# Roy-Shubhajit/FIT-GNN

Measured on AMD Instinct MI355X. Metric: edges aggregated/sec (GCN fwd+bwd) on coarsened subgraphs, higher is better.
Workload: dtype f32

## Files before the change

fit-gnn_amd/csrc/gcn_ops.hip:

```cpp
#include <hip/hip_runtime.h>
#include <stdint.h>

#include <algorithm>

#include "common.h"
#include "fitgnn_hip.h"

namespace {

__global__ void gcn_deg_kernel(const int32_t *__restrict__ rowptr, const float *__restrict__ w, float *__restrict__ dinv,
                               int32_t n_rows) {
    const int i = blockIdx.x * blockDim.x + threadIdx.x;
    if (i >= n_rows) return;
    const int e0 = rowptr[i], e1 = rowptr[i + 1];
    float d = 0.f;
    if (w) {
        for (int e = e0; e < e1; ++e) d += w[e];
    } else {
        d = (float)(e1 - e0);
    }
    dinv[i] = d > 0.f ? 1.0f / sqrtf(d) : 0.f;
}

__global__ void gcn_val_kernel(const int32_t *__restrict__ rowptr, const int32_t *__restrict__ col,
// ... 228 lines not shown
        for (int c = ph; c < n_chunks; c += kColsumPhases) s += partial[(int64_t)c * H + h];
    }
    red[ph][cl] = s;
    __syncthreads();
    for (int w = kColsumPhases / 2; w >= 1; w >>= 1) {
        if (ph < w) red[ph][cl] = red[ph][cl] + red[ph + w][cl];
        __syncthreads();
    }
    if (ph == 0 && h < H) {
        if (db2 && h >= split) db2[h - split] = red[0][cl];
        else if (tr_rows > 0 && h < tr_rows * tr_cols) db[(h % tr_cols) * tr_rows + h / tr_cols] = red[0][cl];
        else db[h] = red[0][cl];
    }
}

__global__ __launch_bounds__(256) void sum_leading_kernel(const float4 *__restrict__ part, int32_t B, int64_t W4,
                                                          float4 *__restrict__ out) {
    const int64_t i = (int64_t)blockIdx.x * 256 + threadIdx.x;
    if (i >= W4) return;
    float4 s[4];
#pragma unroll
    for (int k = 0; k < 4; ++k) s[k] = make_float4(0.f, 0.f, 0.f, 0.f);
    int b = 0;
    for (; b + 4 <= B; b += 4) {
#pragma unroll
        for (int k = 0; k < 4; ++k) {
            const float4 v = part[(int64_t)(b + k) * W4 + i];
            s[k].x += v.x; s[k].y += v.y; s[k].z += v.z; s[k].w += v.w;
        }
    }
// ... 634 lines not shown
    const int blocks = std::min(256, (n_rows + 255) / 256);
    const int rows_per_block = (n_rows + blocks - 1) / blocks;
    const int lds = (kRowTile * row_tile_pitch(C) + 256) * (int)sizeof(float);
    static std::atomic<uint64_t> lds_done{0};
    if (const int rc = fitgnn_lds_limit_once((const void *)narrow_colsum_kernel, (kRowTile * row_tile_pitch(kNarrowMaxC) + 256) * (int)sizeof(float), lds_done)) return rc;
    hipLaunchKernelGGL(narrow_colsum_kernel, dim3(blocks), dim3(256), lds, s, x, ldx, n_rows, C, rows_per_block, (float *)work);
    hipLaunchKernelGGL(colsum_partials_kernel, dim3((C + kColsumCols - 1) / kColsumCols), dim3(kColsumPhases * kColsumCols), 0, s,
                       (const float *)work, blocks, C, out);
    return (int)hipGetLastError();
}

extern "C" int fitgnn_colsum_partials_f32(const float *partial, int32_t n_chunks, int32_t H, float *out, void *stream) {
    if (n_chunks < 1 || H < 1 || !partial || !out) return FITGNN_E_BADARG;
    hipLaunchKernelGGL(colsum_partials_kernel, dim3((H + kColsumCols - 1) / kColsumCols), dim3(kColsumPhases * kColsumCols), 0,
                       (hipStream_t)stream, partial, n_chunks, H, out);
    return (int)hipGetLastError();
}

extern "C" int fitgnn_sum_leading_f32(const float *part, int32_t B, int64_t W, float *out, void *stream) {
    if (B < 1 || W < 0 || (W % 4) != 0) return FITGNN_E_BADARG;
    if (W == 0) return 0;
    if (!part || !out) return FITGNN_E_BADARG;
    if ((((uintptr_t)part | (uintptr_t)out) % 16) != 0) return FITGNN_E_ALIGN;
    const int64_t W4 = W / 4;
    hipLaunchKernelGGL(sum_leading_kernel, dim3((unsigned)((W4 + 255) / 256)), dim3(256), 0, (hipStream_t)stream,
                       (const float4 *)part, B, W4, (float4 *)out);
    return (int)hipGetLastError();
}

extern "C" int fitgnn_gcn_norm_csr_f32(const int32_t *rowptr, const int32_t *col, const float *w, float *val,
// ... 180 lines not shown
```

fit-gnn_amd/csrc/tile_plan.hip:

```cpp
#include <stdint.h>

#include <algorithm>
#include <vector>

#include "fitgnn_hip.h"

namespace {

struct Planner {
    const int32_t *rowptr, *col;
    int32_t max_rows, max_window;
    fitgnn_tile_t *tiles;
    int32_t *win_cols, *lcol;
    int32_t nt = 0, nw = 0;
    std::vector<int32_t> stamp, slot, cur;

    void emit_contiguous(int32_t r0, int32_t r1, int32_t c0, int32_t wn) {
        fitgnn_tile_t t;
        t.row_begin = r0; t.row_end = r1; t.win_begin = c0; t.win_rows = wn;
        t.nnz_begin = rowptr[r0]; t.nnz_end = rowptr[r1];
        t.reserved[0] = 0; t.reserved[1] = 0;
        for (int32_t e = rowptr[r0]; e < rowptr[r1]; ++e) {
            const int32_t s = col[e] - c0;
            lcol[e] = (s >= 0 && s < wn) ? s : -(col[e] + 1);
// ... 146 lines not shown
        rec[0] = (int32_t)r0; rec[1] = (int32_t)r1; rec[2] = rowptr[r0]; rec[3] = rowptr[r1];
        rec[4] = (int32_t)nlong; rec[6] = rec[7] = 0;
        int32_t cnt = 0;
        for (int64_t r = r0; r < r1; ++r)
            if (rowptr[r + 1] - rowptr[r] > long_row) {
                if (nlong >= long_capacity) return FITGNN_E_WORKSPACE;
                long_rows[nlong++] = (int32_t)r;
                ++cnt;
            }
        rec[5] = cnt;
        ++b;
    }
    *n_tiles = nt; *n_large = nl; *n_long = nlong;
    return 0;
}
```

fit-gnn_amd/fitgnn_amd/_lib.py:

```python
import ctypes
import os

_HERE = os.path.dirname(os.path.abspath(__file__))
LIB_PATH = os.path.join(os.path.dirname(_HERE), "lib", "libfitgnn_hip.so")

c_i32, c_i64, c_u32, c_u64, c_f32, c_size = (ctypes.c_int32, ctypes.c_int64, ctypes.c_uint32, ctypes.c_uint64,
                                              ctypes.c_float, ctypes.c_size_t)
ptr = ctypes.c_void_p

EPI_BIAS, EPI_ELU, EPI_DROPOUT, EPI_SEED_DEVICE = 1, 2, 4, 8
SPMM_GATHER = 0x100
MAX_K = 16
MATCH_HEAVY_EDGE, MATCH_ALGEBRAIC_JC = 0, 1
MATCH_SMALL_MAX_NODES, MATCH_SMALL_MAX_NNZ, MATCH_SMALL_MAX_K, MATCH_SMALL_LDS_BUDGET = 128, 1024, 12, 65536
MATCH_DONE, MATCH_TOO_BIG, MATCH_BAD_INPUT = 1, 2, 3
QUALITY_MAX_K = 64

SIGNATURES = {
    "fitgnn_abi_version": (ctypes.c_int, []),
    "fitgnn_error_string": (ctypes.c_char_p, [ctypes.c_int]),
    "fitgnn_stream_copy_f32": (ctypes.c_int, [ptr, ptr, c_i64, ptr]),
    "fitgnn_spmm_default_window_rows": (ctypes.c_int, []),
    "fitgnn_spmm_max_window_rows": (ctypes.c_int, [c_i32]),
    "fitgnn_gcn_norm_csr_f32": (ctypes.c_int, [ptr, ptr, ptr, ptr, ptr, c_i32, ptr]),
# ... 16 lines not shown
    "fitgnn_spmm_csr_stream_dz_f32": (ctypes.c_int, [ptr, ptr, ptr, c_i64, ptr, c_i64, ptr, c_i64, c_i32, c_i32, ptr, c_i32, ptr, c_i32, ptr, ptr,
                                                     ptr, c_u32, c_f32, c_u64, ptr, ptr, ptr]),
    "fitgnn_spmm_rows_compact_parts": (c_i32, [c_i32]),
    "fitgnn_spmm_rows_compact_f32": (ctypes.c_int, [ptr, ptr, ptr, c_i64, ptr, c_i64, c_i32, ptr, c_i64, c_i32, c_i32, ptr]),
    "fitgnn_spmm_rows_compact_dz_f32": (ctypes.c_int, [ptr, ptr, ptr, c_i64, ptr, c_i64, c_i32, ptr, c_i64, c_i32, c_i32, ptr, c_u32, c_f32,
                                                       c_u64, ptr, ptr, ptr]),
    "fitgnn_two_hop_rows_f32": (ctypes.c_int, [ptr, ptr, ptr, ptr, c_i64, c_i32, ptr, c_i32, ptr, c_i32, c_u32, c_f32, c_u64, ptr, ptr, c_i64, ptr]),
    "fitgnn_spmm_two_hop_blocks_f32": (ctypes.c_int, [ptr, ptr, ptr, ptr, c_i64, ptr, c_i64, c_i32, c_i32, ptr, c_i32, ptr, ptr, ptr, ptr, ptr, c_i64,
                                                      c_i32, ptr, ptr, c_u32, c_f32, c_u64, ptr, ptr, ptr]),
    "fitgnn_segment_sum_f32": (ctypes.c_int, [ptr, ptr, c_i32, ptr, c_i64, c_i32, ptr, c_i64, ptr]),
    "fitgnn_segment_max_f32": (ctypes.c_int, [ptr, ptr, c_i32, ptr, c_i64, c_i32, ptr, ptr, ptr]),
    "fitgnn_segment_max_bwd_f32": (ctypes.c_int, [ptr, ptr, c_i32, c_i32, ptr, c_i64, ptr]),
    "fitgnn_segment_expand_f32": (ctypes.c_int, [ptr, ptr, ptr, c_i64, c_i32, ptr, ptr]),
    "fitgnn_make_tiles_host": (ctypes.c_int, [ptr, c_i64, c_i32, ptr, c_i64, ptr]),
    "fitgnn_split_blocks_host": (ctypes.c_int, [ptr, c_i64, ptr, c_i32, c_i64, c_i32, ptr, c_i64, ptr, ptr, ptr, ptr, c_i64, ptr]),
    "fitgnn_plan_tiles_host": (ctypes.c_int, [ptr, ptr, c_i32, c_i32, ptr, c_i32, c_i32, c_i32, ptr, ptr, ptr, ptr, ptr]),
    "fitgnn_epilogue_bwd_workspace_bytes": (c_size, [c_i32, c_i32]),
    "fitgnn_epilogue_bwd_f32": (ctypes.c_int, [ptr, ptr, ptr, c_i32, c_i32, c_u32, c_f32, c_u64, ptr, ptr, ptr, c_size, ptr]),
    "fitgnn_head_max_classes": (ctypes.c_int, []),
    "fitgnn_head_max_classes_wide": (ctypes.c_int, []),
    "fitgnn_epilogue_bwd_head_supported": (ctypes.c_int, [c_i32, c_i32, c_i32]),
    "fitgnn_epilogue_bwd_head_workspace_bytes": (c_size, [c_i32, c_i32, c_i32]),
    "fitgnn_epilogue_bwd_head_f32": (ctypes.c_int, [ptr, ptr, c_i32, ptr, ptr, c_i32, c_i32, c_u32, c_f32, c_u64, ptr, ptr, ptr,
                                                   ptr, c_size, ptr]),
    "fitgnn_epilogue_bwd_head_rows_f32": (ctypes.c_int, [ptr, ptr, c_i32, ptr, ptr, c_i32, c_i32, ptr, c_i32, c_u32, c_f32, c_u64, ptr,
                                                        ptr, ptr, ptr, c_size, ptr]),
    "fitgnn_epilogue_bwd_rows_f32": (ctypes.c_int, [ptr, ptr, ptr, c_i32, c_i32, ptr, c_i32, c_u32, c_f32, c_u64, ptr, ptr, ptr, c_size, ptr]),
    "fitgnn_spmm_epilogue_bwd_supported": (ctypes.c_int, [c_i32, c_i32, c_i32]),
    "fitgnn_spmm_epilogue_bwd_workspace_bytes": (c_size, [c_i32, c_i32, c_i32]),
    "fitgnn_spmm_epilogue_bwd_f32": (ctypes.c_int, [ptr, ptr, ptr, ptr, c_i32, c_i32, ptr, ptr, ptr, c_i32, ptr, ptr, c_i32, c_i32,
# ... 20 lines not shown
    "fitgnn_gemm_exact_workspace_bytes": (c_size, [c_i64, c_i32, c_i64, c_i32, c_i32]),
    "fitgnn_gemm_exact_f32": (ctypes.c_int, [ptr, c_i64, c_i32, ptr, c_i64, c_i32, c_i64, c_i32, c_i64, ptr, c_i64, ptr, ptr]),
    "fitgnn_gemm_exact_plan": (ctypes.c_int, [c_i64, c_i32, c_i64, c_i32, c_i32, ptr, ptr, ptr]),
    "fitgnn_gemm_exact_epi_f32": (ctypes.c_int, [ptr, c_i64, ptr, c_i64, c_i64, c_i32, c_i64, ptr, c_i64, ptr, ptr, c_u32, c_f32, c_u64, ptr, ptr,
                                                 ptr]),
    "fitgnn_gemm_exact_rows_f32": (ctypes.c_int, [ptr, c_i64, c_i32, ptr, ptr, c_i64, c_i32, ptr, c_i64, c_i32, c_i64, ptr, c_i64, ptr, ptr]),
    "fitgnn_gemm_exact_epi_rows_f32": (ctypes.c_int, [ptr, c_i64, ptr, ptr, c_i64, c_i64, c_i32, c_i64, ptr, c_i64, ptr, ptr, c_u32, c_f32,
                                                      c_u64, ptr, ptr, ptr]),
    "fitgnn_gemm_nt_presplit_bytes": (c_size, [c_i32, c_i32]),
    "fitgnn_gemm_nt_presplit_f32": (ctypes.c_int, [ptr, c_i64, c_i64, c_i32, c_i32, c_i32, ptr, ptr]),
    "fitgnn_gemm_nt_pre_f32": (ctypes.c_int, [ptr, c_i64, ptr, c_i64, c_i32, c_i32, ptr, c_i64, ptr]),
    "fitgnn_gemm_nt_epilogue_bwd_workspace_bytes": (c_size, [c_i64, c_i32]),
    "fitgnn_gemm_nt_epilogue_bwd_f32": (ctypes.c_int, [ptr, c_i64, ptr, c_i64, c_i64, c_i32, c_i32, ptr, ptr, ctypes.c_uint32, c_f32,
                                                       ctypes.c_uint64, ptr, ptr, ptr, c_size, ptr]),
    "fitgnn_colsum_partials_f32": (ctypes.c_int, [ptr, c_i32, c_i32, ptr, ptr]),
    "fitgnn_head_rows_lds_bytes": (c_size, [c_i32, c_i32]),
    "fitgnn_head_rows_f32": (ctypes.c_int, [ptr, c_i64, ptr, c_i32, ptr, ptr, c_i32, c_i32, ptr, c_i64, c_i32, ptr]),
    "fitgnn_epilogue_fwd_rows_f32": (ctypes.c_int, [ptr, c_i64, ptr, c_i32, c_i32, ptr, c_u32, c_f32, c_u64, ptr, ptr]),
    "fitgnn_dense_narrow_k_lds_bytes": (c_size, [c_i32, c_i32]),
    "fitgnn_dense_narrow_k_f32": (ctypes.c_int, [ptr, c_i64, ptr, c_i64, c_i32, c_i32, c_i32, ptr, c_u32, c_f32, c_u64, ptr, ptr, c_i64, ptr]),
    "fitgnn_narrow_atb_workspace_bytes": (c_size, [c_i32, c_i32, c_i32]),
    "fitgnn_narrow_atb_f32": (ctypes.c_int, [ptr, c_i64, ptr, c_u32, c_f32, c_u64, ptr, ptr, c_i64, c_i32, c_i32, c_i32, ptr, ptr, ptr, c_size,
                                             ptr]),
    "fitgnn_adam_step_acc_f32": (ctypes.c_int, [ptr, ptr, ptr, ptr, ptr, c_i64, c_f32, c_f32, c_f32, c_f32, c_f32, ptr, ptr, c_i32, c_u64, ptr]),
    "fitgnn_pool_head_supported": (ctypes.c_int, [c_i32, c_i32]),
    "fitgnn_pool_head_f32": (ctypes.c_int, [ptr, ptr, c_i32, ptr, c_i64, c_i32, ptr, ptr, ptr, c_i32, ptr, ptr, ptr]),
    "fitgnn_pool_head_bwd_f32": (ctypes.c_int, [ptr, ptr, c_i32, ptr, ptr, ptr, c_i64, c_i32, c_i32, ptr, ptr, ptr, ptr]),
    "fitgnn_colsum_narrow_workspace_bytes": (c_size, [c_i32, c_i32]),
    "fitgnn_colsum_narrow_f32": (ctypes.c_int, [ptr, c_i64, c_i32, c_i32, ptr, ptr, c_size, ptr]),
    "fitgnn_spmm_narrow_f32": (ctypes.c_int, [ptr, ptr, ptr, ptr, ptr, c_i32, c_i32, c_f32, ptr, c_f32, ptr, c_f32, ptr]),
# ... 179 lines not shown
```

fit-gnn_amd/fitgnn_amd/csr.py:

```python
import ctypes
import weakref

import numpy as np
import torch

from . import _lib

TILE_DTYPE = np.dtype([("row_begin", np.int32), ("row_end", np.int32), ("win_begin", np.int32), ("win_rows", np.int32)])
TILE_INTS = 8


def arrange_tiles_for_xcds(tiles8, n_xcd=8, work=None):
    t = np.ascontiguousarray(tiles8, dtype=np.int32).reshape(-1, TILE_INTS)
    T = t.shape[0]
    if T == 0:
        return t
    if work is None:
        work = (t[:, 1] - t[:, 0]).astype(np.int64) + t[:, 3].astype(np.int64)
    cum = np.concatenate([[0], np.cumsum(work)])
    bounds = np.searchsorted(cum, np.linspace(0, cum[-1], n_xcd + 1), side="left")
    bounds[0], bounds[-1] = 0, T
    bounds = np.maximum.accumulate(bounds)
    L = int(np.max(np.diff(bounds)))
    out = np.zeros((L * n_xcd, TILE_INTS), dtype=np.int32)
# ... 88 lines not shown

def stream_ranges(ptr, n_rows, device, want=8192, min_rows=64):
    ptr = np.asarray(ptr, dtype=np.int64)
    if len(ptr) < 2 or ptr[0] != 0 or ptr[-1] != n_rows:
        raise ValueError("segment boundaries must run from 0 to n_rows")
    ptr = np.unique(ptr)
    n_seg = len(ptr) - 1
    n_ranges = int(max(1, min(want, n_rows // max(min_rows, 1), n_seg)))
    targets = (np.arange(n_ranges + 1, dtype=np.int64) * n_rows) // n_ranges
    rs = np.searchsorted(ptr, targets, side="left")
    rs[0], rs[-1] = 0, n_seg
    rs = np.maximum.accumulate(rs)
    return (torch.from_numpy(ptr.astype(np.int32)).to(device), torch.from_numpy(rs.astype(np.int32)).to(device))


def split_blocks(ptr, rowptr, cap, limit=None):
    ptr = np.ascontiguousarray(ptr, dtype=np.int64)
    rp = np.ascontiguousarray(rowptr.detach().cpu().numpy() if torch.is_tensor(rowptr) else rowptr, dtype=np.int32)
    nb = len(ptr) - 1
    n = int(ptr[-1])
    if limit is None:
        limit = max(4 * cap, n // 2048)
    t_cap = nb + n // max(int(cap), 1) + 2
    tiles4 = np.zeros((t_cap, 4), dtype=np.int32)
    blocks = np.zeros((max(nb, 1), BLOCK_INTS), dtype=np.int32)
    longs = np.zeros(max(n, 1), dtype=np.int32)
    nt, nl, nlong = ctypes.c_int64(0), ctypes.c_int64(0), ctypes.c_int64(0)
    _lib.call("fitgnn_split_blocks_host", ptr.ctypes.data, nb, rp.ctypes.data, int(cap), int(limit), LONG_ROW, tiles4.ctypes.data, t_cap,
              ctypes.byref(nt), blocks.ctypes.data, ctypes.byref(nl), longs.ctypes.data, len(longs), ctypes.byref(nlong))
    small = np.zeros(nt.value, dtype=TILE_DTYPE)
    if nt.value:
        arr = tiles4[: nt.value]
        small["row_begin"], small["row_end"], small["win_begin"], small["win_rows"] = arr[:, 0], arr[:, 1], arr[:, 2], arr[:, 3]
    blocks = blocks[: nl.value].copy()
    long_rows = longs[: nlong.value].copy()
    if nl.value:
        blocks = arrange_tiles_for_xcds(blocks, work=(blocks[:, 1] - blocks[:, 0]).astype(np.int64))
    return small, blocks, long_rows


def split_blocks_py(ptr, rowptr, cap, limit=None):
    ptr = np.asarray(ptr, dtype=np.int64)
    rp = rowptr.detach().cpu().numpy().astype(np.int64)
    size = np.diff(ptr)
    if limit is None:
        limit = max(4 * cap, int(ptr[-1]) // 2048)
    is_large = (size > cap) & (size <= limit)
    large = np.nonzero(is_large)[0]
    tiles = []
    nb = len(size)
    b = 0
    while b < nb:
        if is_large[b]:
# ... 53 lines not shown
    win = np.zeros(max(nnz, 1), dtype=np.int32)
    lcol = np.zeros(max(nnz, 1), dtype=np.int32)
    nt, nw = ctypes.c_int32(0), ctypes.c_int32(0)
    bp, nb = None, 0
    if block_ptr is not None:
        bp = np.ascontiguousarray(block_ptr.detach().cpu().numpy() if torch.is_tensor(block_ptr) else block_ptr, dtype=np.int64)
        nb = len(bp) - 1
    _lib.call("fitgnn_plan_tiles_host", rp.ctypes.data, cc.ctypes.data, n_rows, n_rows, None if bp is None else bp.ctypes.data, nb, int(max_rows),
              int(max_window), tiles.ctypes.data, ctypes.byref(nt), win.ctypes.data, ctypes.byref(nw), lcol.ctypes.data)
    return tiles[: nt.value].copy(), win[: max(nw.value, 1)].copy(), lcol[: max(nnz, 1)].copy()


class CSRGraph:

    def __init__(self, edge_index, num_nodes, mode="gcn", ptr=None, lds_rows=None, planned=False, gather=False, split_large=True,
                 block_limit=None):
        assert edge_index.dim() == 2 and edge_index.shape[0] == 2
        device = edge_index.device
        self.device, self.n, self.mode = device, int(num_nodes), mode
        self.planned, self.gather, self.split_large, self.block_limit = planned, gather, split_large, block_limit
        self.split_min_rows = 600_000
        self.fold_ok = (not planned) and (not gather)
        src, dst = edge_index[0].to(torch.int64), edge_index[1].to(torch.int64)
        if mode in ("gcn", "gat"):
            keep = src != dst
            loop = torch.arange(self.n, device=device, dtype=torch.int64)
            src, dst = torch.cat([src[keep], loop]), torch.cat([dst[keep], loop])
        rowptr, col, _ = _csr_from_coo(dst, src, self.n)
        self.nnz = int(col.numel())
        counts = (rowptr[1:] - rowptr[:-1]).to(torch.int64)
        rows_f = torch.repeat_interleave(torch.arange(self.n, device=device), counts)
        rowptr_t, col_t, self._perm_t = _csr_from_coo(col.to(torch.int64), rows_f, self.n)
        self.f, self.t = _Side(rowptr, col), _Side(rowptr_t, col_t)
        self.dinv = None
        self.seg = self.range_seg = None
# ... 39 lines not shown
        if self.planned:
            for side in (f, t):
                tiles, win, lcol = plan_tiles(side.rowptr, side.col, self.n, cap, cap, block_ptr=ptr_np if len(ptr_np) > 2 else None)
                side.tiles = torch.from_numpy(arrange_tiles_for_xcds(tiles)).to(dev)
                side.win_cols = torch.from_numpy(win).to(dev)
                side.lcol = torch.from_numpy(lcol).to(dev)
                side.n_tiles = int(tiles.shape[0])
        else:
            tiles = make_tiles(ptr_np, cap)
            has_large = bool(len(ptr_np) > 1 and np.max(np.diff(ptr_np)) > cap)
            for side in (f, t):
                rp_host = np.ascontiguousarray(side.rowptr.detach().cpu().numpy(), dtype=np.int32)
                side.tiles = tiles_to_device(tiles, side.rowptr, rp_host)
                side.n_tiles = int(tiles.shape[0])
                if has_large and self.split_large and not self.gather and self.nnz > 0:
                    small, blocks, long_rows = split_blocks(ptr_np, rp_host, cap, self.block_limit)
                    in_blocks = int((blocks[:, 1] - blocks[:, 0]).sum()) if len(blocks) else 0
                    if self.block_limit is None and (in_blocks * 5 < self.n * 3 or self.n < self.split_min_rows):
                        continue
                    side.small_tiles = tiles_to_device(small, side.rowptr, rp_host) if len(small) else torch.zeros((0, TILE_INTS), dtype=torch.int32, device=dev)
                    side.blocks = torch.from_numpy(blocks).to(dev)
                    side.long_rows = torch.from_numpy(long_rows if len(long_rows) else np.zeros(1, dtype=np.int32)).to(dev)
                    if self.seg is None:
                        self.seg, self.range_seg = stream_ranges(ptr_np, self.n, dev)
        return self


_CACHE = {}


def csr_for(edge_index, num_nodes, mode="gcn"):
    key = (edge_index.data_ptr(), int(edge_index._version), tuple(edge_index.shape), int(num_nodes), mode,
# ... 66 lines not shown
```

fit-gnn_amd/fitgnn_amd/ops.py:

```python
import ctypes

import os

import torch

from . import _lib
from ._lib import EPI_BIAS, EPI_DROPOUT, EPI_ELU


class OpConfig:
    __slots__ = ("gemm_precision", "atb_kernel", "nt_kernel", "nt_presplit", "fuse_dx_epilogue", "fold_backward",
                 "dedup_gather", "pad_table_min_k", "split_large_blocks", "compact_head_backward", "last_layer_on_loss_rows",
                 "compact_rows_kernel", "stream_kernel", "two_hop_backward", "narrow_input_first", "fused_pool_head", "fused_gemm_epilogue", "rows_in_gemm", "pooled_rows_last_layer", "rows_kernel_min_rows", "appnp_in_lds", "appnp_blocks", "appnp_sliced", "grad_sink", "profile", "profile_gemm",
                 "profile_fused", "seed_bank")

    def __init__(self, gemm_precision="exact", atb_kernel=True, nt_kernel=True, nt_presplit=True, fuse_dx_epilogue=True,
                 fold_backward=False, dedup_gather=True, pad_table_min_k=0, split_large_blocks=True, compact_head_backward=True,
                 last_layer_on_loss_rows=True, compact_rows_kernel=True, stream_kernel=False, two_hop_backward=True, narrow_input_first=True, fused_pool_head=True, fused_gemm_epilogue=True, rows_in_gemm=True, pooled_rows_last_layer=True, rows_kernel_min_rows=32768, appnp_in_lds=True, appnp_blocks=True, appnp_sliced=True, grad_sink=None,
                 profile=None, profile_gemm=None, profile_fused=None, seed_bank=None):
        if gemm_precision not in ("exact", "high", "highest"):
            raise ValueError(f"gemm_precision {gemm_precision!r}: 'exact', 'high' or 'highest'")
        self.gemm_precision, self.atb_kernel, self.nt_kernel, self.nt_presplit = gemm_precision, atb_kernel, nt_kernel, nt_presplit
        self.fuse_dx_epilogue, self.fold_backward, self.dedup_gather = fuse_dx_epilogue, fold_backward, dedup_gather
        self.pad_table_min_k, self.split_large_blocks = pad_table_min_k, split_large_blocks
        self.compact_head_backward, self.last_layer_on_loss_rows = compact_head_backward, last_layer_on_loss_rows
        self.compact_rows_kernel, self.stream_kernel, self.two_hop_backward = compact_rows_kernel, stream_kernel, two_hop_backward
        self.narrow_input_first, self.fused_pool_head, self.grad_sink = narrow_input_first, fused_pool_head, grad_sink
        self.fused_gemm_epilogue, self.rows_in_gemm = fused_gemm_epilogue, rows_in_gemm
        self.pooled_rows_last_layer, self.rows_kernel_min_rows = pooled_rows_last_layer, int(rows_kernel_min_rows)
        self.appnp_in_lds, self.appnp_blocks, self.appnp_sliced = appnp_in_lds, appnp_blocks, appnp_sliced
        self.profile, self.profile_gemm, self.profile_fused, self.seed_bank = profile, profile_gemm, profile_fused, seed_bank

    def replace(self, **kw):
        cur = {k: getattr(self, k) for k in self.__slots__}
# ... 582 lines not shown
    Y = torch.empty((g.n, H), dtype=torch.float32, device=dev)
    st = _lib.stream_ptr(dev)
    n_seg, n_ranges = int(g.seg.numel()) - 1, int(g.range_seg.numel()) - 1
    seed_v, epi_v = _seed_arg(seed, epilogue)
    db = None
    with _timed(cfg, kind or ("dz" if dz is not None else ("tile" if xrow is None else "table"))):
        if dz is None:
            _lib.call("fitgnn_spmm_csr_stream_f32", side.rowptr, side.col, side.val, int(side.col.numel()), Xc, Xc.stride(0), Y, Y.stride(0), g.n,
                      H, g.seg, n_seg, g.range_seg, n_ranges, xrow, xcol, bias, epi_v, float(p), seed_v, mask, st)
        else:
            prev, want_db = dz
            part = torch.empty((n_ranges, H), dtype=torch.float32, device=dev) if want_db else None
            _lib.call("fitgnn_spmm_csr_stream_dz_f32", side.rowptr, side.col, side.val, int(side.col.numel()), Xc, Xc.stride(0), Y, Y.stride(0),
                      g.n, H, g.seg, n_seg, g.range_seg, n_ranges, xrow, xcol, prev, epi_v, float(p), seed_v, mask, part, st)
            if want_db:
                db = _fold_partials(part, dev, st)
    return Y if dz is None else (Y, db)


def _spmm_rows_compact(g, side, Xc, xrow, zero_from, cfg, kind, dz=None, val=None):
    _lib.require_cuda(Xc, xrow)
    val = side.val if val is None else val
    H, dev = Xc.shape[1], Xc.device
    xcol = _entry_rows(side, xrow)
    Y = torch.empty((g.n, H), dtype=torch.float32, device=dev)
    st = _lib.stream_ptr(dev)
    db = None
    with _timed(cfg, kind or ("compact" if dz is None else "compact_dz")):
        if dz is None:
            _lib.call("fitgnn_spmm_rows_compact_f32", side.rowptr, xcol, val, int(side.col.numel()), Xc, Xc.stride(0), int(zero_from), Y,
                      Y.stride(0), g.n, H, st)
        else:
            prev, epilogue, p, seed, mask, want_db = dz
            seed_v, epi_v = _seed_arg(seed, epilogue & ~_lib.SPMM_GATHER)
            n_part = int(_lib.lib().fitgnn_spmm_rows_compact_parts(g.n))
            part = torch.empty((n_part, H), dtype=torch.float32, device=dev) if want_db else None
            _lib.call("fitgnn_spmm_rows_compact_dz_f32", side.rowptr, xcol, val, int(side.col.numel()), Xc, Xc.stride(0), int(zero_from), Y,
                      Y.stride(0), g.n, H, prev, epi_v, float(p), seed_v, mask, part, st)
            if want_db:
                db = _fold_partials(part, dev, st)
    return Y if dz is None else (Y, db)


def two_hop_supported(g, link, Xc, prev, cfg):
    return (cfg.two_hop_backward and link is not None and link.g is g and Xc.shape[1] % 4 == 0 and prev.is_contiguous()
            and prev.shape[1] == Xc.shape[1] and g.t.blocks is not None and cfg.split_large_blocks)


NO_ROW = 0x7fffffff


BLOCK_PIECE_ROWS = 16
BLOCK_CARRIED = 4


# ... 53 lines not shown
    H, dev = Xc.shape[1], Xc.device
    n_sel = int(rows.numel())
    ix = _two_hop_block_index(g, rows, pos)
    n_zt = int(ix["zt_rows"].numel())
    seed_v, epi_v = _seed_arg(link.seed, link.epi)
    st = _lib.stream_ptr(dev)
    with _timed(cfg, profile_kind or "two_hop"):
        ZT = torch.empty((max(n_zt, 1), H), dtype=torch.float32, device=dev)
        _lib.call("fitgnn_two_hop_rows_f32", side.rowptr, ix["zcol"], side.val, Xc, Xc.stride(0), n_sel, ix["zt_rows"], n_zt, prev, H, epi_v,
                  float(link.p), seed_v, link.mask, ZT, ZT.stride(0), st)
        Y = torch.empty((g.n, H), dtype=torch.float32, device=dev)
        quiet = cfg if cfg.profile is None else cfg.replace(profile=None)
        if side.small_tiles.shape[0]:
            spmm_raw(side.rowptr, side.col, side.val, side.small_tiles, ZT, g.n, window_rows=g.window_rows, out=Y, cfg=quiet, xrow=ix["zrow"])
        n_blocks = int(side.blocks.shape[0])
        part = _scratch((n_blocks + 1, H), dev) if link.want_db else None
        _lib.call("fitgnn_spmm_two_hop_blocks_f32", side.rowptr, side.col, side.val, ZT, ZT.stride(0), Y, Y.stride(0), g.n, H, side.blocks, n_blocks,
                  side.long_rows, ix["zrow"], ix["zcol"], prev, Xc, Xc.stride(0), n_sel, ix["row_p"], ix["row_w"], epi_v, float(link.p), seed_v,
                  link.mask, part, st)
        db = None
        if link.want_db:
            if ix["tile_zt"].numel():
                torch.sum(ZT.index_select(0, ix["tile_zt"]), 0, out=part[n_blocks])
            else:
                part[n_blocks].zero_()
            db = _fold_partials(part, dev, st)
    return Y, db


def _fold_partials(part, dev, st):
    n_part, H = int(part.shape[0]), int(part.shape[1])
    if n_part > 8192:
        G = 1024
        per = n_part // G
        head = part[: G * per].view(G, per, H).sum(1)
        part = torch.cat([head, part[G * per:]]) if n_part > G * per else head
        n_part = int(part.shape[0])
    db = torch.empty(H, dtype=torch.float32, device=dev)
    _lib.call("fitgnn_colsum_partials_f32", part.contiguous(), n_part, H, db, st)
    return db


def spmm_graph_dz(g, X, prev, epilogue, p=0.0, seed=0, mask=None, want_db=True, transposed=True, xrow=None, cfg=DEFAULT, profile_kind=None,
                  zero_from=-1):
    side = g.t if transposed else g.f
    Xc, prev = _f32c(X), _f32c(prev)
# ... 13 lines not shown
    n_blocks = int(side.blocks.shape[0]) if split else 0
    Y = torch.empty((g.n, H), dtype=torch.float32, device=dev)
    part = _scratch((n_tiles + n_blocks, H), dev) if want_db else None
    st = _lib.stream_ptr(dev)
    with _timed(cfg, profile_kind or "dz"):
        if n_tiles:
            _lib.call("fitgnn_spmm_csr_dz_f32", side.rowptr, side.col, side.val, Xc, Xc.stride(0), Y, Y.stride(0), g.n, H, tiles, n_tiles,
                      None if split else side.lcol, None if split else side.win_cols, xrow, int(zero_from), int(g.window_rows), prev, epi_v, float(p),
                      seed_v, mask, part, st)
        if n_blocks:
            xcol = None
            if xrow is not None:
                xcol = _entry_rows(side, xrow)
            _lib.call("fitgnn_spmm_csr_blocks_dz_f32", side.rowptr, side.col, side.val, Xc, Xc.stride(0), Y, Y.stride(0), g.n, H, side.blocks, n_blocks,
                      side.long_rows, xrow, xcol, int(zero_from), prev, epi_v, float(p), seed_v, mask, None if part is None else part[n_tiles:], st)
    db = _fold_partials(part, dev, st) if want_db else None
    return Y, db


def epilogue_bwd_head_raw(dy, Wl, out, epilogue, p=0.0, seed=0, mask=None, want_db=True, want_dWl=True):
    _lib.require_cuda(dy, Wl, out, mask)
    L = _lib.lib()
    dy, Wl, out = _f32c(dy), _f32c(Wl), _f32c(out)
    n, H = out.shape
    C = Wl.shape[0]
    seed, epilogue = _seed_arg(seed, epilogue)
    dZ = torch.empty_like(out)
    db = torch.empty(H, dtype=torch.float32, device=out.device) if want_db else None
    dWl = torch.empty((C, H), dtype=torch.float32, device=out.device) if want_dWl else None
    wb = int(L.fitgnn_epilogue_bwd_head_workspace_bytes(n, H, C))
    work = torch.empty(max(wb, 4), dtype=torch.uint8, device=out.device)
# ... 1480 lines not shown
```

include/fitgnn_hip.h:

```cpp
#ifndef FITGNN_HIP_H
#define FITGNN_HIP_H

#include <stddef.h>
#include <stdint.h>

#ifdef __cplusplus
extern "C" {
#endif

#define FITGNN_ABI_VERSION 1
#define FITGNN_MAX_K 16

#define FITGNN_E_BADARG (-1)
#define FITGNN_E_WORKSPACE (-2)
#define FITGNN_E_ALIGN (-3)

int fitgnn_abi_version(void);
const char *fitgnn_error_string(int code);

int fitgnn_stream_copy_f32(const float *src, float *dst, int64_t n, void *stream);


typedef struct fitgnn_tile {
    int32_t row_begin, row_end;
    int32_t win_begin;
    int32_t win_rows;
    int32_t nnz_begin, nnz_end;
    int32_t reserved[2];
} fitgnn_tile_t;

int fitgnn_plan_tiles_host(const int32_t *rowptr, const int32_t *col, int32_t n_rows, int32_t n_cols,
                           const int64_t *block_ptr, int32_t n_blocks, int32_t max_rows, int32_t max_window,
                           fitgnn_tile_t *tiles, int32_t *n_tiles, int32_t *win_cols, int32_t *n_win, int32_t *lcol);

int fitgnn_make_tiles_host(const int64_t *ptr, int64_t n_blocks, int32_t max_rows, int32_t *tiles4, int64_t capacity, int64_t *n_tiles);
int fitgnn_split_blocks_host(const int64_t *ptr, int64_t n_blocks, const int32_t *rowptr, int32_t cap, int64_t limit, int32_t long_row,
                             int32_t *tiles4, int64_t tiles_capacity, int64_t *n_tiles, int32_t *blocks8, int64_t *n_large,
                             int32_t *long_rows, int64_t long_capacity, int64_t *n_long);

typedef struct fitgnn_block {
    int32_t row_begin, row_end;
    int32_t nnz_begin, nnz_end;
    int32_t long_off, n_long;
    int32_t reserved[2];
} fitgnn_block_t;

int fitgnn_spmm_csr_blocks_f32(const int32_t *rowptr, const int32_t *col, const float *val, const float *X, int64_t ldx,
                               float *Y, int64_t ldy, int32_t n_rows, int32_t H, const fitgnn_block_t *blocks,
                               int32_t n_blocks, const int32_t *long_rows, const int32_t *xrow, const int32_t *xcol,
// ... 114 lines not shown

size_t fitgnn_gemm_nt_epilogue_bwd_workspace_bytes(int64_t R, int32_t N);
int fitgnn_gemm_nt_epilogue_bwd_f32(const float *a, int64_t lda, const float *b, int64_t ldb, int64_t R, int32_t N, int32_t K,
                                    const float *out, float *dZ, uint32_t epilogue, float p_drop, uint64_t seed,
                                    const uint8_t *mask, float *db, void *work, size_t work_bytes, void *stream);

size_t fitgnn_head_rows_lds_bytes(int32_t H, int32_t C);
int fitgnn_head_rows_f32(const float *out, int64_t ldo, const int64_t *rows, int32_t n_rows, const float *Wl, const float *bl,
                         int32_t C, int32_t H, float *y, int64_t ldy, int32_t out_compact, void *stream);

size_t fitgnn_colsum_narrow_workspace_bytes(int32_t n_rows, int32_t C);
int fitgnn_colsum_narrow_f32(const float *x, int64_t ldx, int32_t n_rows, int32_t C, float *out, void *work, size_t work_bytes,
                             void *stream);

int fitgnn_colsum_partials_f32(const float *partial, int32_t n_chunks, int32_t H, float *out, void *stream);

int fitgnn_l1_loss_f32(const float *out, const float *tgt, int32_t n, float scale, float *loss, float *grad, void *stream);

size_t fitgnn_softmax_nll_workspace_bytes(int32_t n);
int fitgnn_softmax_nll_f32(const float *z, int64_t ldz, int32_t n_rows, int32_t C, const int64_t *idx,
                           const int64_t *labels, int32_t n, float scale, float *loss, float *dz, void *work,
                           size_t work_bytes, void *stream);

int fitgnn_adam_step_f32(float *param, const float *grad, float *exp_avg, float *exp_avg_sq, int64_t n, float lr,
                         float beta1, float beta2, float eps, float weight_decay, float *step, void *stream);

int fitgnn_adam_step_acc_f32(float *param, float *grad_acc, float *grad_new, float *exp_avg, float *exp_avg_sq, int64_t n, float lr,
                             float beta1, float beta2, float eps, float weight_decay, float *state, uint64_t *seeds, int32_t n_seeds,
                             uint64_t seed_stride, void *stream);

// ... 307 lines not shown
```

Baseline: 3.636 billion.

## Fold bias-gradient partials in one ticketed kernel and route small star tiles as blocks

Adds a single-pass column-sum kernel that splits the partial rows into up to 1024 runs and sums each run with Kahan summation. The last block to finish each column slab, detected with an atomic ticket, folds the run results into the bias gradient. This replaces the earlier multi-step fold used when there are more than 8192 partials. Small contiguous tiles inside small star blocks can now also be turned into block records for the block SpMM path, and the tile/block split heuristic now counts only oversized blocks. The cost is an atomic ticket protocol with a tickets buffer that must be reset, and changed routing that may shift load between the tile and block kernels.

```diff
diff --git a/fit-gnn_amd/csrc/gcn_ops.hip b/fit-gnn_amd/csrc/gcn_ops.hip
--- a/fit-gnn_amd/csrc/gcn_ops.hip
+++ b/fit-gnn_amd/csrc/gcn_ops.hip
@@ -266,6 +266,65 @@
     }
 }
 
+__device__ __forceinline__ void kahan_add(float &s, float &comp, float v) {
+    const float y = v - comp;
+    const float t = s + y;
+    comp = (t - s) - y;
+    s = t;
+}
+constexpr int kRunsMax = 1024, kRunCols = 256, kRunBatch = 16, kRunFoldBatch = 64;
+__global__ __launch_bounds__(kRunCols) void colsum_partials_runs_kernel(const float *__restrict__ partial, int32_t n, int32_t H, int32_t per,
+                                                                         int32_t n_runs, int32_t n_slabs, float *scratch, unsigned *tickets,
+                                                                         float *__restrict__ out) {
+    __shared__ int s_last;
+    const int run = blockIdx.x / n_slabs, slab = blockIdx.x % n_slabs;
+    const int h = slab * kRunCols + (int)threadIdx.x;
+    if (h < H) {
+        const int r0 = run * per, r1 = min(n, r0 + per);
+        const float *p = partial + (int64_t)r0 * H + h;
+        float s = 0.f, comp = 0.f;
+        int r = r0;
+        for (; r + kRunBatch <= r1; r += kRunBatch) {
+            float v[kRunBatch];
+#pragma unroll
+            for (int u = 0; u < kRunBatch; ++u) v[u] = p[(int64_t)u * H];
+#pragma unroll
+            for (int u = 0; u < kRunBatch; ++u) kahan_add(s, comp, v[u]);
+            p += (int64_t)kRunBatch * H;
+        }
+        if (r < r1) {
+            float v[kRunBatch];
+#pragma unroll
+            for (int u = 0; u < kRunBatch; ++u) v[u] = p[(int64_t)min(u, r1 - 1 - r) * H];
+#pragma unroll
+            for (int u = 0; u < kRunBatch; ++u)
+                if (r + u < r1) kahan_add(s, comp, v[u]);
+        }
+        __hip_atomic_store(scratch + (int64_t)run * H + h, s, __ATOMIC_RELAXED, __HIP_MEMORY_SCOPE_AGENT);
+    }
+    asm volatile("s_waitcnt vmcnt(0)" ::: "memory");
+    __syncthreads();
+    if (threadIdx.x == 0)
+        s_last = __hip_atomic_fetch_add(&tickets[slab], 1u, __ATOMIC_RELAXED, __HIP_MEMORY_SCOPE_AGENT) == (unsigned)n_runs - 1u;
+    __syncthreads();
+    if (!s_last) return;
+    if (h < H) {
+        const float *q = scratch + h;
+        float s = 0.f, comp = 0.f;
+        for (int k = 0; k < n_runs; k += kRunFoldBatch) {
+            float v[kRunFoldBatch];
+#pragma unroll
+            for (int u = 0; u < kRunFoldBatch; ++u)
+                v[u] = __hip_atomic_load(q + (int64_t)min(k + u, n_runs - 1) * H, __ATOMIC_RELAXED, __HIP_MEMORY_SCOPE_AGENT);
+#pragma unroll
+            for (int u = 0; u < kRunFoldBatch; ++u)
+                if (k + u < n_runs) kahan_add(s, comp, v[u]);
+        }
+        out[h] = s;
+    }
+    if (threadIdx.x == 0) tickets[slab] = 0u;
+}
+
 __global__ __launch_bounds__(256) void sum_leading_kernel(const float4 *__restrict__ part, int32_t B, int64_t W4,
                                                           float4 *__restrict__ out) {
     const int64_t i = (int64_t)blockIdx.x * 256 + threadIdx.x;
@@ -930,6 +989,23 @@
     if (n_chunks < 1 || H < 1 || !partial || !out) return FITGNN_E_BADARG;
     hipLaunchKernelGGL(colsum_partials_kernel, dim3((H + kColsumCols - 1) / kColsumCols), dim3(kColsumPhases * kColsumCols), 0,
                        (hipStream_t)stream, partial, n_chunks, H, out);
+    return (int)hipGetLastError();
+}
+
+extern "C" int32_t fitgnn_colsum_partials_runs_count(int32_t n) {
+    if (n < 1) return 0;
+    const int32_t per = (n + kRunsMax - 1) / kRunsMax;
+    return (n + per - 1) / per;
+}
+
+extern "C" int fitgnn_colsum_partials_runs_f32(const float *partial, int32_t n, int32_t H, float *out, float *scratch, uint32_t *tickets,
+                                               void *stream) {
+    if (n < 1 || H < 1 || !partial || !out || !scratch || !tickets) return FITGNN_E_BADARG;
+    const int32_t per = (n + kRunsMax - 1) / kRunsMax, n_runs = (n + per - 1) / per;
+    const int32_t n_slabs = (H + kRunCols - 1) / kRunCols;
+    if ((int64_t)n_runs * n_slabs > 0x7fffffff) return FITGNN_E_BADARG;
+    hipLaunchKernelGGL(colsum_partials_runs_kernel, dim3((unsigned)(n_runs * n_slabs)), dim3(kRunCols), 0, (hipStream_t)stream, partial, n, H,
+                       per, n_runs, n_slabs, scratch, (unsigned *)tickets, out);
     return (int)hipGetLastError();
 }
 
diff --git a/fit-gnn_amd/csrc/tile_plan.hip b/fit-gnn_amd/csrc/tile_plan.hip
--- a/fit-gnn_amd/csrc/tile_plan.hip
+++ b/fit-gnn_amd/csrc/tile_plan.hip
@@ -184,3 +184,33 @@
     *n_tiles = nt; *n_large = nl; *n_long = nlong;
     return 0;
 }
+
+extern "C" int fitgnn_tiles_as_blocks_host(const int64_t *ptr, int64_t n_blocks, const int32_t *rowptr, int32_t cap, int64_t limit,
+                                           const int32_t *tiles4, int64_t n_tiles, int32_t *blocks8, int64_t *n_records, int32_t *kept4,
+                                           int64_t *n_kept) {
+    if (n_blocks < 0 || n_tiles < 0 || cap < 1 || !n_records || !n_kept) return FITGNN_E_BADARG;
+    *n_records = *n_kept = 0;
+    if (n_tiles == 0) return 0;
+    if (!ptr || !rowptr || !tiles4 || !blocks8 || !kept4 || n_blocks == 0) return FITGNN_E_BADARG;
+    int64_t nr = 0, nk = 0;
+    for (int64_t i = 0; i < n_tiles; ++i) {
+        const int32_t *t = tiles4 + 4 * i;
+        const int64_t r0 = t[0], r1 = t[1];
+        if (r0 < ptr[0] || r1 > ptr[n_blocks] || r1 < r0) return FITGNN_E_BADARG;
+        bool ok = r1 > r0 && t[2] == t[0] && (int64_t)t[3] == r1 - r0 && r1 - r0 <= cap;
+        if (ok) {
+            const int64_t b = (std::upper_bound(ptr, ptr + n_blocks + 1, r0) - ptr) - 1;
+            ok = b < n_blocks && ptr[b + 1] - ptr[b] <= limit;
+        }
+        if (ok) {
+            int32_t *rec = blocks8 + 8 * nr++;
+            rec[0] = t[0]; rec[1] = t[1]; rec[2] = rowptr[r0]; rec[3] = rowptr[r1];
+            rec[4] = rec[5] = rec[6] = rec[7] = 0;
+        } else {
+            int32_t *k = kept4 + 4 * nk++;
+            k[0] = t[0]; k[1] = t[1]; k[2] = t[2]; k[3] = t[3];
+        }
+    }
+    *n_records = nr; *n_kept = nk;
+    return 0;
+}
diff --git a/fit-gnn_amd/fitgnn_amd/_lib.py b/fit-gnn_amd/fitgnn_amd/_lib.py
--- a/fit-gnn_amd/fitgnn_amd/_lib.py
+++ b/fit-gnn_amd/fitgnn_amd/_lib.py
@@ -54,6 +54,7 @@
     "fitgnn_segment_expand_f32": (ctypes.c_int, [ptr, ptr, ptr, c_i64, c_i32, ptr, ptr]),
     "fitgnn_make_tiles_host": (ctypes.c_int, [ptr, c_i64, c_i32, ptr, c_i64, ptr]),
     "fitgnn_split_blocks_host": (ctypes.c_int, [ptr, c_i64, ptr, c_i32, c_i64, c_i32, ptr, c_i64, ptr, ptr, ptr, ptr, c_i64, ptr]),
+    "fitgnn_tiles_as_blocks_host": (ctypes.c_int, [ptr, c_i64, ptr, c_i32, c_i64, ptr, c_i64, ptr, ptr, ptr, ptr]),
     "fitgnn_plan_tiles_host": (ctypes.c_int, [ptr, ptr, c_i32, c_i32, ptr, c_i32, c_i32, c_i32, ptr, ptr, ptr, ptr, ptr]),
     "fitgnn_epilogue_bwd_workspace_bytes": (c_size, [c_i32, c_i32]),
     "fitgnn_epilogue_bwd_f32": (ctypes.c_int, [ptr, ptr, ptr, c_i32, c_i32, c_u32, c_f32, c_u64, ptr, ptr, ptr, c_size, ptr]),
@@ -104,6 +105,8 @@
     "fitgnn_gemm_nt_epilogue_bwd_f32": (ctypes.c_int, [ptr, c_i64, ptr, c_i64, c_i64, c_i32, c_i32, ptr, ptr, ctypes.c_uint32, c_f32,
                                                        ctypes.c_uint64, ptr, ptr, ptr, c_size, ptr]),
     "fitgnn_colsum_partials_f32": (ctypes.c_int, [ptr, c_i32, c_i32, ptr, ptr]),
+    "fitgnn_colsum_partials_runs_count": (c_i32, [c_i32]),
+    "fitgnn_colsum_partials_runs_f32": (ctypes.c_int, [ptr, c_i32, c_i32, ptr, ptr, ptr, ptr]),
     "fitgnn_head_rows_lds_bytes": (c_size, [c_i32, c_i32]),
     "fitgnn_head_rows_f32": (ctypes.c_int, [ptr, c_i64, ptr, c_i32, ptr, ptr, c_i32, c_i32, ptr, c_i64, c_i32, ptr]),
     "fitgnn_epilogue_fwd_rows_f32": (ctypes.c_int, [ptr, c_i64, ptr, c_i32, c_i32, ptr, c_u32, c_f32, c_u64, ptr, ptr]),
diff --git a/fit-gnn_amd/fitgnn_amd/csr.py b/fit-gnn_amd/fitgnn_amd/csr.py
--- a/fit-gnn_amd/fitgnn_amd/csr.py
+++ b/fit-gnn_amd/fitgnn_amd/csr.py
@@ -126,7 +126,7 @@
     return (torch.from_numpy(ptr.astype(np.int32)).to(device), torch.from_numpy(rs.astype(np.int32)).to(device))
 
 
-def split_blocks(ptr, rowptr, cap, limit=None):
+def split_blocks(ptr, rowptr, cap, limit=None, small_stars_as_blocks=False):
     ptr = np.ascontiguousarray(ptr, dtype=np.int64)
     rp = np.ascontiguousarray(rowptr.detach().cpu().numpy() if torch.is_tensor(rowptr) else rowptr, dtype=np.int32)
     nb = len(ptr) - 1
@@ -146,9 +146,39 @@
         small["row_begin"], small["row_end"], small["win_begin"], small["win_rows"] = arr[:, 0], arr[:, 1], arr[:, 2], arr[:, 3]
     blocks = blocks[: nl.value].copy()
     long_rows = longs[: nlong.value].copy()
-    if nl.value:
+    if small_stars_as_blocks and len(small):
+        records, small = tiles_as_blocks(ptr, rp, cap, limit, small)
+        blocks = np.concatenate([blocks, records])
+        blocks = blocks[np.argsort(blocks[:, 0], kind="stable")]
+    if len(blocks):
         blocks = arrange_tiles_for_xcds(blocks, work=(blocks[:, 1] - blocks[:, 0]).astype(np.int64))
     return small, blocks, long_rows
+
+
+def tiles_as_blocks(ptr, rowptr, cap, limit, tiles):
+    ptr = np.ascontiguousarray(ptr, dtype=np.int64)
+    rp = np.ascontiguousarray(rowptr, dtype=np.int32)
+    t4 = np.ascontiguousarray(tiles).view(np.int32).reshape(-1, 4)
+    nt = t4.shape[0]
+    records = np.zeros((max(nt, 1), BLOCK_INTS), dtype=np.int32)
+    kept4 = np.zeros((max(nt, 1), 4), dtype=np.int32)
+    nr, nk = ctypes.c_int64(0), ctypes.c_int64(0)
+    _lib.call("fitgnn_tiles_as_blocks_host", ptr.ctypes.data, len(ptr) - 1, rp.ctypes.data, int(cap), int(limit), t4.ctypes.data, nt,
+              records.ctypes.data, ctypes.byref(nr), kept4.ctypes.data, ctypes.byref(nk))
+    return records[: nr.value].copy(), kept4[: nk.value].copy().view(TILE_DTYPE).reshape(-1)
+
+
+def tiles_as_blocks_py(ptr, rowptr, cap, limit, tiles):
+    ptr = np.asarray(ptr, dtype=np.int64)
+    rp = np.asarray(rowptr, dtype=np.int64)
+    t4 = np.ascontiguousarray(tiles).view(np.int32).reshape(-1, 4).astype(np.int64)
+    r0, r1 = t4[:, 0], t4[:, 1]
+    block = np.searchsorted(ptr, r0, side="right") - 1
+    size = ptr[np.minimum(block + 1, len(ptr) - 1)] - ptr[block]
+    ok = (r1 > r0) & (t4[:, 2] == r0) & (t4[:, 3] == r1 - r0) & (r1 - r0 <= cap) & (block < len(ptr) - 1) & (size <= limit)
+    records = np.zeros((int(ok.sum()), BLOCK_INTS), dtype=np.int32)
+    records[:, 0], records[:, 1], records[:, 2], records[:, 3] = r0[ok], r1[ok], rp[r0[ok]], rp[r1[ok]]
+    return records, np.ascontiguousarray(t4[~ok].astype(np.int32)).view(TILE_DTYPE).reshape(-1)
 
 
 def split_blocks_py(ptr, rowptr, cap, limit=None):
@@ -232,11 +262,12 @@
 class CSRGraph:
 
     def __init__(self, edge_index, num_nodes, mode="gcn", ptr=None, lds_rows=None, planned=False, gather=False, split_large=True,
-                 block_limit=None):
+                 block_limit=None, small_stars_as_blocks=None):
         assert edge_index.dim() == 2 and edge_index.shape[0] == 2
         device = edge_index.device
         self.device, self.n, self.mode = device, int(num_nodes), mode
         self.planned, self.gather, self.split_large, self.block_limit = planned, gather, split_large, block_limit
+        self.small_stars_as_blocks = (block_limit is None) if small_stars_as_blocks is None else bool(small_stars_as_blocks)
         self.split_min_rows = 600_000
         self.fold_ok = (not planned) and (not gather)
         src, dst = edge_index[0].to(torch.int64), edge_index[1].to(torch.int64)
@@ -306,8 +337,9 @@
                 side.tiles = tiles_to_device(tiles, side.rowptr, rp_host)
                 side.n_tiles = int(tiles.shape[0])
                 if has_large and self.split_large and not self.gather and self.nnz > 0:
-                    small, blocks, long_rows = split_blocks(ptr_np, rp_host, cap, self.block_limit)
-                    in_blocks = int((blocks[:, 1] - blocks[:, 0]).sum()) if len(blocks) else 0
+                    small, blocks, long_rows = split_blocks(ptr_np, rp_host, cap, self.block_limit, self.small_stars_as_blocks)
+                    rows_of = blocks[:, 1] - blocks[:, 0]
+                    in_blocks = int(rows_of[rows_of > cap].sum()) if len(blocks) else 0
                     if self.block_limit is None and (in_blocks * 5 < self.n * 3 or self.n < self.split_min_rows):
                         continue
                     side.small_tiles = tiles_to_device(small, side.rowptr, rp_host) if len(small) else torch.zeros((0, TILE_INTS), dtype=torch.int32, device=dev)
diff --git a/fit-gnn_amd/fitgnn_amd/ops.py b/fit-gnn_amd/fitgnn_amd/ops.py
--- a/fit-gnn_amd/fitgnn_amd/ops.py
+++ b/fit-gnn_amd/fitgnn_amd/ops.py
@@ -12,12 +12,13 @@
     __slots__ = ("gemm_precision", "atb_kernel", "nt_kernel", "nt_presplit", "fuse_dx_epilogue", "fold_backward",
                  "dedup_gather", "pad_table_min_k", "split_large_blocks", "compact_head_backward", "last_layer_on_loss_rows",
                  "compact_rows_kernel", "stream_kernel", "two_hop_backward", "narrow_input_first", "fused_pool_head", "fused_gemm_epilogue", "rows_in_gemm", "pooled_rows_last_layer", "rows_kernel_min_rows", "appnp_in_lds", "appnp_blocks", "appnp_sliced", "grad_sink", "profile", "profile_gemm",
-                 "profile_fused", "seed_bank")
+                 "profile_fused", "seed_bank", "native_partial_fold")
 
     def __init__(self, gemm_precision="exact", atb_kernel=True, nt_kernel=True, nt_presplit=True, fuse_dx_epilogue=True,
                  fold_backward=False, dedup_gather=True, pad_table_min_k=0, split_large_blocks=True, compact_head_backward=True,
                  last_layer_on_loss_rows=True, compact_rows_kernel=True, stream_kernel=False, two_hop_backward=True, narrow_input_first=True, fused_pool_head=True, fused_gemm_epilogue=True, rows_in_gemm=True, pooled_rows_last_layer=True, rows_kernel_min_rows=32768, appnp_in_lds=True, appnp_blocks=True, appnp_sliced=True, grad_sink=None,
-                 profile=None, profile_gemm=None, profile_fused=None, seed_bank=None):
+                 profile=None, profile_gemm=None, profile_fused=None, seed_bank=None, native_partial_fold=True):
+        self.native_partial_fold = native_partial_fold
         if gemm_precision not in ("exact", "high", "highest"):
             raise ValueError(f"gemm_precision {gemm_precision!r}: 'exact', 'high' or 'highest'")
         self.gemm_precision, self.atb_kernel, self.nt_kernel, self.nt_presplit = gemm_precision, atb_kernel, nt_kernel, nt_presplit
@@ -630,7 +631,7 @@
             _lib.call("fitgnn_spmm_csr_stream_dz_f32", side.rowptr, side.col, side.val, int(side.col.numel()), Xc, Xc.stride(0), Y, Y.stride(0),
                       g.n, H, g.seg, n_seg, g.range_seg, n_ranges, xrow, xcol, prev, epi_v, float(p), seed_v, mask, part, st)
             if want_db:
-                db = _fold_partials(part, dev, st)
+                db = _fold_partials(part, dev, st, cfg, g)
     return Y if dz is None else (Y, db)
 
 
@@ -654,7 +655,7 @@
             _lib.call("fitgnn_spmm_rows_compact_dz_f32", side.rowptr, xcol, val, int(side.col.numel()), Xc, Xc.stride(0), int(zero_from), Y,
                       Y.stride(0), g.n, H, prev, epi_v, float(p), seed_v, mask, part, st)
             if want_db:
-                db = _fold_partials(part, dev, st)
+                db = _fold_partials(part, dev, st, cfg, g)
     return Y if dz is None else (Y, db)
 
 
@@ -738,22 +739,39 @@
         if side.small_tiles.shape[0]:
             spmm_raw(side.rowptr, side.col, side.val, side.small_tiles, ZT, g.n, window_rows=g.window_rows, out=Y, cfg=quiet, xrow=ix["zrow"])
         n_blocks = int(side.blocks.shape[0])
-        part = _scratch((n_blocks + 1, H), dev) if link.want_db else None
+        extra = 1 if ix["tile_zt"].numel() else 0
+        part = _scratch((n_blocks + extra, H), dev) if link.want_db else None
         _lib.call("fitgnn_spmm_two_hop_blocks_f32", side.rowptr, side.col, side.val, ZT, ZT.stride(0), Y, Y.stride(0), g.n, H, side.blocks, n_blocks,
                   side.long_rows, ix["zrow"], ix["zcol"], prev, Xc, Xc.stride(0), n_sel, ix["row_p"], ix["row_w"], epi_v, float(link.p), seed_v,
                   link.mask, part, st)
         db = None
         if link.want_db:
-            if ix["tile_zt"].numel():
+            if extra:
                 torch.sum(ZT.index_select(0, ix["tile_zt"]), 0, out=part[n_blocks])
-            else:
-                part[n_blocks].zero_()
-            db = _fold_partials(part, dev, st)
+            db = _fold_partials(part, dev, st, cfg, g)
     return Y, db
 
 
-def _fold_partials(part, dev, st):
+def fold_partials_runs(part, owner=None, st=None):
+    _lib.require_cuda(part)
+    part = _f32c(part)
+    n_part, H, dev = int(part.shape[0]), int(part.shape[1]), part.device
+    n_slabs = (H + 255) // 256
+    tickets = getattr(owner, "_fold_tickets", None)
+    if tickets is None or tickets.numel() < n_slabs or tickets.device != dev:
+        tickets = torch.zeros(max(8, n_slabs), dtype=torch.int32, device=dev)
+        if owner is not None:
+            owner._fold_tickets = tickets
+    runs = _scratch((int(_lib.lib().fitgnn_colsum_partials_runs_count(n_part)), H), dev)
+    db = torch.empty(H, dtype=torch.float32, device=dev)
+    _lib.call("fitgnn_colsum_partials_runs_f32", part, n_part, H, db, runs, tickets, _lib.stream_ptr(dev) if st is None else st)
+    return db
+
+
+def _fold_partials(part, dev, st, cfg=DEFAULT, owner=None):
     n_part, H = int(part.shape[0]), int(part.shape[1])
+    if n_part > 8192 and cfg.native_partial_fold:
+        return fold_partials_runs(part, owner, st)
     if n_part > 8192:
         G = 1024
         per = n_part // G
@@ -797,7 +815,7 @@
                 xcol = _entry_rows(side, xrow)
             _lib.call("fitgnn_spmm_csr_blocks_dz_f32", side.rowptr, side.col, side.val, Xc, Xc.stride(0), Y, Y.stride(0), g.n, H, side.blocks, n_blocks,
                       side.long_rows, xrow, xcol, int(zero_from), prev, epi_v, float(p), seed_v, mask, None if part is None else part[n_tiles:], st)
-    db = _fold_partials(part, dev, st) if want_db else None
+    db = _fold_partials(part, dev, st, cfg, g) if want_db else None
     return Y, db
 
 
diff --git a/include/fitgnn_hip.h b/include/fitgnn_hip.h
--- a/include/fitgnn_hip.h
+++ b/include/fitgnn_hip.h
@@ -33,6 +33,8 @@
                            const int64_t *block_ptr, int32_t n_blocks, int32_t max_rows, int32_t max_window,
                            fitgnn_tile_t *tiles, int32_t *n_tiles, int32_t *win_cols, int32_t *n_win, int32_t *lcol);
 
+int fitgnn_tiles_as_blocks_host(const int64_t *ptr, int64_t n_blocks, const int32_t *rowptr, int32_t cap, int64_t limit, const int32_t *tiles4,
+                                int64_t n_tiles, int32_t *blocks8, int64_t *n_records, int32_t *kept4, int64_t *n_kept);
 int fitgnn_make_tiles_host(const int64_t *ptr, int64_t n_blocks, int32_t max_rows, int32_t *tiles4, int64_t capacity, int64_t *n_tiles);
 int fitgnn_split_blocks_host(const int64_t *ptr, int64_t n_blocks, const int32_t *rowptr, int32_t cap, int64_t limit, int32_t long_row,
                              int32_t *tiles4, int64_t tiles_capacity, int64_t *n_tiles, int32_t *blocks8, int64_t *n_large,
@@ -177,6 +179,10 @@
                              void *stream);
 
 int fitgnn_colsum_partials_f32(const float *partial, int32_t n_chunks, int32_t H, float *out, void *stream);
+
+int32_t fitgnn_colsum_partials_runs_count(int32_t n);
+int fitgnn_colsum_partials_runs_f32(const float *partial, int32_t n, int32_t H, float *out, float *scratch, uint32_t *tickets,
+                                    void *stream);
 
 int fitgnn_l1_loss_f32(const float *out, const float *tgt, int32_t n, float scale, float *loss, float *grad, void *stream);
 
```

Result: no change. 3.647 billion (median of 6 runs) (+0.3%).
